# EdwardsLabProjects/sequence-alignment-tools

Measured on AMD Instinct MI355X. Metric: Gbases/s scanned, 100k×20-mer primers k≤2, 3 Gbp DB at 1/2/4/8 GPUs, higher is better.
Workload: dtype u32

## Files before the change

### sequence-alignment-tools_amd/csrc/pm_api.cpp

```cpp
#include <algorithm>
#include <climits>
#include <cstdio>
#include <cstring>
#include <memory>
#include <new>
#include <chrono>
#include <thread>
#include <unordered_map>

#include "pm_internal.h"
#include "pm_iupac.h"
#include "pm_seed.h"
#include "pm_pair.h"

using namespace pm;

namespace pm {
void Alphabet::set_raw() {
  size = 256;
  for (int i = 0; i < 256; ++i) { ch[i] = (uint8_t)i; nch[i] = i; present[i] = true; }
}
void Alphabet::set_table(const uint8_t *table, int len) {
  size = len;
  for (int i = 0; i < 256; ++i) { ch[i] = 0; nch[i] = -1; present[i] = true; }
// ... 1406 lines not shown
extern "C" int pm_reset(pm_handle *h) {
  if (!h) return PM_E_INVALID;
  drain_spec(h);
  if (h->scan_pending) { (void)hipStreamSynchronize(h->stream); h->scan_pending = false; }
  h->carry.clear(); h->land_n = h->land_pos = 0; h->next_begin = 0;
  std::fill(h->lasthit.begin(), h->lasthit.end(), 0);
  h->halves_fresh = true;
  h->last_count = 0;
  h->scan_mode = 0;
  return count_clear(h);
}

extern "C" void pm_destroy(pm_handle *h) {
  if (!h) return;
  (void)hipSetDevice(h->cfg.device);
  free_device(h);
  delete h;
}

extern "C" const char *pm_last_error(const pm_handle *h) { return h ? h->err.c_str() : g_create_error.c_str(); }
extern "C" int pm_selected_semantics(const pm_handle *h) { return h && h->inited ? h->sem : PM_E_INVALID; }
extern "C" int pm_selected_kernel(const pm_handle *h) { return h && h->inited ? h->kern : PM_E_INVALID; }

static const char *pair_schedule_name(const ScanGeometry &g) {
  return g.work_map == PAIR_MAP_XCD_SUPERCHUNK ? "xcd-superchunk" : g.work_map == PAIR_MAP_XCD ? "xcd" : "superchunk";
}

extern "C" int pm_describe(const pm_handle *h, char *buf, size_t buflen) {
  if (!h || !buf || !h->inited) return PM_E_INVALID;
  if (h->kern == PM_KERNEL_SEED && h->short_only)
    snprintf(buf, buflen, "kernel=pm_short_edit_scan+pm_edits_verify for %zu patterns of 16..19 characters (tiles=%d, tests=%d) fields=2-of-4 x 4 bases, displaced by |d| <= %d window=16 chunk=%lld nchunks=%d grid=%d block=%d",
             h->nshort, (int)h->shd.tiles.size(), h->shd.k == 2 ? SHORT_NTESTS : 2, h->shd.k, (long long)h->geo.seg_len, h->geo.nseg, h->geo.blocks, h->geo.threads);
  else if (h->kern == PM_KERNEL_SEED && !h->pair.empty()) {
    snprintf(buf, buflen, "kernel=pm_pair_scan tiles=%d combos=%d fields=2-of-4 x 5 bases window=20 row_slots=%d chunk=%lld nchunks=%d grid=%d block=%d lds=%d schedule=%s",
             (int)h->pair.size(), h->pair[0].ncombos, h->pair[0].stride, (long long)h->geo.seg_len, h->geo.nseg, h->geo.blocks, h->geo.threads, PAIR_LDS_BYTES,
             pair_schedule_name(h->geo));
    if (h->nlong) {
      int wide = 0;
      for (const PairDevice &d : h->pair) wide += d.wide ? 1 : 0;
      const size_t at = strlen(buf);
      if (at < buflen) snprintf(buf + at, buflen - at, " with %zu patterns of 33..64 characters (pm_pair_verify_wide, wide tiles=%d)", h->nlong, wide);
    }
    if (h->nrest) {
      const size_t at = strlen(buf);
      if (at < buflen) snprintf(buf + at, buflen - at, " + %s for %zu patterns the seed plan does not take", bitpar_kernel_name(h->scan_k, h->scan_indels), h->nrest);
    }
  }
  else if (h->kern == PM_KERNEL_SEED && h->edits_dev && h->epair_on) {
    snprintf(buf, buflen, "kernel=pm_pair_edit_scan+pm_pair_edit_resolve+pm_edits_verify tiles=1 tests=14 fields=2-of-4 x 5 bases, displaced by |d| <= 2 window=20 row_slots=%d slot_patterns=2 chunk=%lld nchunks=%d grid=%d block=%d lds=%d schedule=%s",
             h->epair.stride, (long long)h->geo.seg_len, h->geo.nseg, h->geo.blocks, h->geo.threads, PAIR_LDS_BYTES, pair_schedule_name(h->geo));
    if (h->nrest) {
      const size_t at = strlen(buf);
      if (at < buflen) snprintf(buf + at, buflen - at, " + %s for %zu patterns the seed plan does not take", bitpar_kernel_name(h->scan_k, h->scan_indels), h->nrest);
    }
  }
  else if (h->kern == PM_KERNEL_SEED) {
    snprintf(buf, buflen, "kernel=%s tiles=%d combos=%d pieces=%d-of-%d x %d bases window=%d slots=%zu chunk=%lld nchunks=%d grid=%d block=%d lds=%d",
             h->sd.edits && h->sd.edit_tabulated ? "pm_edit_scan+pm_edits_verify" : h->sd.edits ? "pm_seed_scan+pm_edits_verify" :
             h->sd.halves && h->sd.half_ranked ? "pm_half_scan+pm_half_verify" : "pm_seed_scan", 1 + (int)h->sd_more.size(), h->sd.ncombos, h->sd.r, h->sd.k + h->sd.r, h->sd.pb, h->sd.Lw, h->sd.nslots, (long long)h->geo.seg_len, h->geo.nseg,
             h->geo.blocks, h->geo.threads, SEED_LDS_BYTES);
    if (h->nlong_exact) {
      int wide = h->sd.wide ? 1 : 0;
      for (const SeedDevice &d : h->sd_more) wide += d.wide ? 1 : 0;
      const size_t at = strlen(buf);
      if (at < buflen) snprintf(buf + at, buflen - at, " with %zu patterns of 33..64 characters (wide rows, wide tiles=%d)", h->nlong_exact, wide);
    }
    if (h->nrest) {
      const size_t at = strlen(buf);
      if (at < buflen) snprintf(buf + at, buflen - at, " + %s for %zu patterns the seed plan does not take", bitpar_kernel_name(h->scan_k, h->scan_indels), h->nrest);
    }
  }
  if (h->kern == PM_KERNEL_SEED && h->nshort && !h->short_only) {
    const size_t at = strlen(buf);
    if (at < buflen) snprintf(buf + at, buflen - at, " + pm_short_edit_scan for %zu patterns of 16..19 characters (tiles=%d, tests=%d)", h->nshort, (int)h->shd.tiles.size(), h->shd.k == 2 ? SHORT_NTESTS : 2);
  }
  if (h->kern == PM_KERNEL_SEED && h->nssub) {
    const size_t at = strlen(buf);
    if (at < buflen) snprintf(buf + at, buflen - at, " + pm_short_sub_scan for %zu patterns of 16..19 characters (tiles=%d, pairs=%d)", h->nssub, (int)h->ssd.tiles.size(), h->ssd.ncombos);
  }
  if (h->kern == PM_KERNEL_SEED) return PM_OK;
  else
    snprintf(buf, buflen, "kernel=%s tiles=%d lanes_per_tile=64 words_per_lane=%d seg_len=%lld nseg=%d grid=%d block=%d",
             bitpar_kernel_name(h->scan_k, h->scan_indels), h->bp.ntiles, BP_WPL, (long long)h->geo.seg_len, h->geo.nseg,
// ... 1736 lines not shown
```

### sequence-alignment-tools_amd/csrc/pm_pair.h

```cpp
#pragma once
#include <array>
#include <cstdint>
#include <string>
#include <vector>

#include "pm_internal.h"
#include "pm_workmap.h"

namespace pm {

constexpr int PAIR_THREADS = 1024;
constexpr int PAIR_WAVES = PAIR_THREADS / 64;
constexpr int PAIR_MAX_COMBOS = 6;
constexpr int PAIR_BITMAP_WORDS = 32768;
constexpr int PAIR_QUEUE = 128;
constexpr int PAIR_LDS_BYTES = PAIR_BITMAP_WORDS * 4 + PAIR_WAVES * PAIR_QUEUE * 16;
static_assert(PAIR_LDS_BYTES <= 163840, "160 KiB of LDS per workgroup");
constexpr int PAIR_XCD_MIN_CHUNKS = 5 * 256;

struct PairTables {
  int k = 0, maxlen = 0, ncombos = 0, eos_code = -1, stride = 0;
  bool ascii = false;
  bool wide = false;
  int fa[PAIR_MAX_COMBOS] = {}, fb[PAIR_MAX_COMBOS] = {};
  std::vector<uint32_t> image;
  std::vector<uint64_t> slots;
  std::vector<uint32_t> row_base;
  std::vector<uint32_t> first_pat;
  std::vector<uint32_t> order;
  std::vector<uint32_t> olist;
  size_t first_off[PAIR_MAX_COMBOS] = {};
  std::vector<uint64_t> pat40;
  std::vector<uint8_t> pat_len;
  std::vector<uint32_t> pat_id;
  std::vector<uint8_t> pat_codes;
  std::vector<uint32_t> pat_zone;
};

struct PairDevice {
  int k = 0, maxlen = 0, ncombos = 0, eos_code = -1, stride = 0;
  bool ascii = false;
  bool wide = false;
  int fa[PAIR_MAX_COMBOS] = {}, fb[PAIR_MAX_COMBOS] = {};
  size_t first_off[PAIR_MAX_COMBOS] = {};
  size_t np = 0;
  uint64_t *slots = nullptr;
  uint32_t *image = nullptr, *row_base = nullptr, *first_pat = nullptr, *order = nullptr, *olist = nullptr, *pat_id = nullptr;
  uint64_t *pat40 = nullptr;
  uint8_t *pat_len = nullptr, *pat_codes = nullptr;
  uint32_t *pat_zone = nullptr;
  int viol_level = 0;
  Knobs knobs;
};

constexpr int PAIR_MAX_LEN = 32, PAIR_MAX_LEN_WIDE = 64;
std::string pair_build(const std::vector<Pattern> &pats, const std::vector<uint32_t> &ids, const Alphabet &alpha, int k,
                       int eos_code, PairTables *out, int stride_knob = 0, int slot_patterns = 3, int max_len = PAIR_MAX_LEN);
hipError_t pair_upload(const PairTables &t, PairDevice *d, hipStream_t st);
void pair_free(PairDevice *d);
ScanGeometry pair_geometry(const PairDevice &d, int64_t begin, int64_t end);
constexpr size_t PAIR_SUSPECT_BYTES = 16;
hipError_t pair_launch(const PairDevice &d, const uint8_t *d_text, const uint32_t *d_packed, int64_t n, int64_t begin, int64_t end,
                       pm_hit *d_out, unsigned long long *d_counter, uint64_t cap, void *d_susp, unsigned long long *d_susp_count, uint64_t susp_cap,
                       hipStream_t st, ScanGeometry *geo_out, unsigned long long *d_stats = nullptr, int floor_mode = 0,
                       uint64_t *seed_out = nullptr, unsigned long long *seed_count = nullptr, uint64_t seed_cap = 0);

}
```

### sequence-alignment-tools_amd/csrc/pm_pair.hip

```cpp
#include "pm_bits.h"
#include "pm_internal.h"
#include "pm_pair.h"
#include "pm_verify.h"
#include "pm_workmap.h"

#include <algorithm>
#include <cstring>
#include <thread>
#include <type_traits>
#include <utility>

namespace pm {

namespace {

constexpr int WAVES = PAIR_WAVES;
constexpr uint32_t F20 = 0xfffffu;
constexpr uint32_t WHAT_REST = 8u, WHAT_ALL = 16u;
__device__ __host__ __forceinline__ uint64_t slot_pack(uint32_t o1, uint32_t o2, uint32_t o3, bool walk) {
  return (uint64_t)o1 | ((uint64_t)o2 << 20) | ((uint64_t)o3 << 40) | ((uint64_t)(walk ? 8 : 0) << 60);
}

struct PairArgs {
  const uint8_t *text;
  int64_t n, begin, end;
  const uint32_t *packed;
  int64_t npacked;
  int64_t chunk0, chunk_len;
  int nchunks, ncombos, group;
  int work_map;
  int k, eos_code, debug;
  int stride;
  int fa[PAIR_MAX_COMBOS], fb[PAIR_MAX_COMBOS];
  const uint32_t *image;
  const uint2 *slots;
  const uint32_t *row_base;
  const uint32_t *first_pat, *order;
  const uint32_t *olist;
  uint32_t first_off[PAIR_MAX_COMBOS];
  uint32_t np;
  const uint2 *pat40;
  const uint8_t *pat_len;
  const uint32_t *pat_id;
  const uint8_t *pat_codes;
  const uint32_t *pat_zone;
  int viol_level;
  pm_hit *out;
  unsigned long long *counter;
  unsigned long long cap;
  uint4 *susp;
  unsigned long long *susp_count;
  unsigned long long susp_cap;
  uint64_t *seed_out;
  unsigned long long *seed_count;
  unsigned long long seed_cap;
  unsigned long long *stats;
};

typedef __attribute__((address_space(3))) uint32_t lds_u32;
typedef uint32_t u32x4 __attribute__((ext_vector_type(4)));
typedef uint32_t u32x2 __attribute__((ext_vector_type(2)));
typedef __attribute__((address_space(3))) u32x4 lds_u128;
__device__ __forceinline__ lds_u128 *lds128(uint32_t addr) { return reinterpret_cast<lds_u128 *>((uintptr_t)addr); }
__device__ __forceinline__ lds_u32 *lds32(uint32_t addr) { return reinterpret_cast<lds_u32 *>((uintptr_t)addr); }

__device__ __host__ __forceinline__ uint32_t field_of(uint64_t W, int j) { return (uint32_t)(W >> (10 * j)) & 0x3ffu; }
__device__ __host__ __forceinline__ void other_fields(int a, int b, int *c, int *d) {
  int o[2], t = 0;
  for (int j = 0; j < 4; ++j) if (j != a && j != b) o[t++] = j;
  *c = o[0]; *d = o[1];
}


template <int OFF>
__device__ __forceinline__ uint32_t wbits(uint32_t wlo, uint32_t whi) {
  static_assert(OFF >= 0 && OFF < 48, "window offset");
  if constexpr (OFF == 0) return wlo;
  else if constexpr (OFF < 32) return __builtin_amdgcn_alignbit(whi, wlo, OFF);
  else return whi >> (OFF - 32);
}
template <int NB, int T>
__device__ __forceinline__ uint32_t mism(uint32_t p, uint32_t wlo, uint32_t whi) {
  static_assert(T >= -2 && T + NB <= 22, "text base outside the window");
  const uint32_t x = p ^ wbits<2 * (T + 2)>(wlo, whi);
  return (x | (x >> 1)) & (NB == 5 ? 0x155u : 0x55555u);
}
enum { REG_L = 0, REG_M = 1, REG_R = 2 };
template <int NB>
__device__ __forceinline__ bool two_deletions(uint32_t lowm, uint32_t midm, uint32_t highm) {
  const int lo = __builtin_ctz(lowm | (1u << (2 * NB)));
  const int hi = 31 - __builtin_clz(highm | 1u);
  const uint32_t between = ((1u << hi) - 1u) & ~((2u << lo) - 1u);
  return (midm & between) == 0;
}
template <int KIND, int NB, int T0, int BASE, int DSP, int BUDGET>
// ... 90 lines not shown
__device__ __host__ __forceinline__ int edit_variant_table(int var) { return var == 0 ? 0 : (var <= 3 ? 1 : (var <= 8 ? 2 : (var == 9 ? 3 : (var <= 12 ? 4 : 5)))); }


template <int CW>
__device__ __forceinline__ void pair_resolve(const PairArgs &a, const VerifyStage &vs, int combo, uint32_t rank, uint32_t what, uint32_t wo, int64_t p, pm_hit *first, bool *have) {
  const uint32_t *fp = a.first_pat + a.first_off[combo];
  const uint32_t *ord = a.order + (size_t)combo * a.np;
  const uint32_t *ol = a.olist + (size_t)combo * a.np;
  const uint32_t t0 = fp[rank], t1 = fp[rank + 1];
  pm_hit hh;
  auto take = [&](bool ok) __attribute__((always_inline)) {
    const bool extra = ok && *have;
    if (ok && !*have) { *first = hh; *have = true; }
    pair_emit(a, vs, extra, hh);
  };
  for (uint32_t j = 0; j < 3; ++j)
    take(((what >> j) & 1u) && t0 + j < t1 && pair_verify<5, CW>(a, combo, p, ord[t0 + j], &hh));
  if (what & (WHAT_REST | WHAT_ALL)) {
    for (uint32_t t = t0 + ((what & WHAT_ALL) ? 0u : 3u); t < t1; ++t)
      take(sym_distance(ol[t] ^ wo) <= a.k && pair_verify<5, CW>(a, combo, p, ord[t], &hh));
  }
}

template <int CW>
__device__ __forceinline__ void pair_verify_body(const PairArgs &a) {
  unsigned long long n = *a.susp_count;
  if (n > a.susp_cap) n = a.susp_cap;
  verify_staged(a, n, [&](unsigned long long i, const VerifyStage &vs, pm_hit *first) __attribute__((always_inline)) {
    bool have = false;
    const uint4 r = a.susp[i];
    const uint64_t pw = ((uint64_t)r.w << 32) | r.z;
    if (r.x != 0xffffffffu) {
      const int combo = (int)((pw >> 40) & 7u);
      const uint32_t key = r.x, wo = r.y, row = key & 0x7fffu, bit = key >> 15;
      const uint32_t wd = a.image[(size_t)combo * PAIR_BITMAP_WORDS + row];
      if ((wd >> bit) & 1u) {
        const uint32_t lr = (uint32_t)__popc(wd & ((1u << bit) - 1u));
        const uint32_t rank = a.row_base[(size_t)combo * (PAIR_BITMAP_WORDS + 1) + row] + lr;
        uint32_t what = WHAT_ALL;
        if (lr < (uint32_t)a.stride - 1u) {
          const uint2 sl = a.slots[((size_t)combo * PAIR_BITMAP_WORDS + row) * (size_t)a.stride + lr];
          const uint64_t S = ((uint64_t)sl.y << 32) | sl.x;
          what = (sym_distance(((uint32_t)S ^ wo) & F20) <= a.k ? 1u : 0u) | (sym_distance(((uint32_t)(S >> 20) ^ wo) & F20) <= a.k ? 2u : 0u) |
                 (sym_distance(((uint32_t)(S >> 40) ^ wo) & F20) <= a.k ? 4u : 0u) | ((sl.y >> 31) ? WHAT_REST : 0u);
        }
        pair_resolve<CW>(a, vs, combo, rank, what, wo, (int64_t)(pw & 0xffffffffffull), first, &have);
      }
    }
    return have && !(a.debug & 16);
  });
}
__global__ __launch_bounds__(256) void pm_pair_verify(PairArgs a) { pair_verify_body<32>(a); }
__global__ __launch_bounds__(256) void pm_pair_verify_wide(PairArgs a) { pair_verify_body<64>(a); }

template <int A, int B, int DSP = 0, int FLOOR = 0>
__device__ __forceinline__ void pair_scan_body(const PairArgs &a, const int combo, const int cj, const int variant = 0) {
  constexpr int C = (A != 0 && B != 0) ? 0 : ((A != 1 && B != 1) ? 1 : 2);
  constexpr int D = (A != 3 && B != 3) ? 3 : ((A != 2 && B != 2) ? 2 : 1);
  static_assert(A < B && C < D && C != A && C != B && D != A && D != B, "fields");
  const int lane = threadIdx.x & 63;
  const int wave = __builtin_amdgcn_readfirstlane((int)(threadIdx.x >> 6));
  const int64_t sub = a.chunk_len / WAVES;
  const int64_t ws = (a.chunk0 + cj) * a.chunk_len + (int64_t)wave * sub;
  int64_t own_lo = ws > a.begin ? ws : a.begin;
  int64_t own_hi = ws + sub;
  if (own_hi > a.end) own_hi = a.end;
  if (own_hi > a.n) own_hi = a.n;
  if (own_lo < 19) own_lo = 19;
  if (own_lo >= own_hi) return;

  const uint32_t stride = (uint32_t)a.stride, kmax = stride - 1u;
  const char *slots = reinterpret_cast<const char *>(a.slots + (size_t)combo * PAIR_BITMAP_WORDS * stride);
  uint32_t carry1, carry2;
  {
    const uint32_t pk = load_packed(a.packed, a.npacked, ws - 32 + 16 * (lane & 1));
    carry2 = __builtin_amdgcn_readlane(pk, 0);
    carry1 = __builtin_amdgcn_readlane(pk, 1);
  }
  const uint32_t QB = PAIR_BITMAP_WORDS * 4 + (uint32_t)wave * (PAIR_QUEUE * 16);
  int qn = 0;
  uint32_t keep = 0;

  const int64_t pre_hi = FLOOR == 3 ? own_hi + 1024 : own_hi;
  uint32_t q0 = load_packed(a.packed, a.npacked, ws + 16 * lane);
  uint32_t q1 = ws + 1024 < pre_hi ? load_packed(a.packed, a.npacked, ws + 1024 + 16 * lane) : 0u;
  uint32_t q2 = ws + 2048 < pre_hi ? load_packed(a.packed, a.npacked, ws + 2048 + 16 * lane) : 0u;
  uint32_t q3 = ws + 3072 < pre_hi ? load_packed(a.packed, a.npacked, ws + 3072 + 16 * lane) : 0u;
  const uint32_t *pk_wave = a.packed + (ws >> 4);
  uint32_t pf_idx = 4096u / 16u + (uint32_t)lane;

  const int negk1 = -(a.k + 1);

  unsigned long long blk_at = 0;
  uint32_t blk_left = 0, blk_next = 0;
  auto flush = [&]() __attribute__((always_inline)) {
    int done = 0;
    while (done < qn) {
      if (blk_left == 0) {
        const uint32_t want = max((uint32_t)(qn - done), blk_next);
        unsigned long long base = 0;
        if (lane == 0) base = atomicAdd(a.susp_count, (unsigned long long)want);
        blk_at = ((unsigned long long)__builtin_amdgcn_readfirstlane((uint32_t)(base >> 32)) << 32) | __builtin_amdgcn_readfirstlane((uint32_t)base);
        blk_left = want;
        blk_next = min(2u * max(want, 64u), 4096u);
      }
// ... 13 lines not shown
    blk_left = 0;
  };
  auto enqueue = [&](bool mine, uint32_t key, uint32_t wo, uint32_t prel) __attribute__((always_inline)) {
    const unsigned long long bal = __ballot(mine);
    if (bal == 0) return;
    if (a.debug & 1) { keep ^= key; return; }
    if (mine) {
      const int s_ = qn + (int)__builtin_amdgcn_mbcnt_hi((uint32_t)(bal >> 32), __builtin_amdgcn_mbcnt_lo((uint32_t)bal, 0));
      u32x4 q;
      q.x = key; q.y = wo; q.z = prel; q.w = 0;
      *lds128(QB + 16 * (uint32_t)s_) = q;
    }
    qn += __popcll(bal);
    if (qn >= 64) flush();
  };

  auto key_of = [&](auto WIN, uint32_t prev2, uint32_t prev1, uint32_t cur) __attribute__((always_inline)) -> uint32_t {
    constexpr int I = decltype(WIN)::value;
    const uint32_t X = bits_at<2 * I + 26 + 10 * A - 2 - 2 * DSP>(prev2, prev1, cur);
    if constexpr (B == A + 1 && DSP == 0) return X;
    else { const uint32_t Y = bits_at<2 * I + 26 + 10 * B - 12>(prev2, prev1, cur); return (X & 0xffcu) | (Y & ~0xffcu); }
  };

#ifndef PM_PAIR_NR
#define PM_PAIR_NR 6
#endif
  constexpr int NR = PM_PAIR_NR;
  static_assert(NR % 2 == 0 && NR >= 4 && NR <= 12, "ring size");
  uint32_t P = 0;
  uint32_t pu1 = 0, pu2 = 0, pu3 = 0, cu1 = 0, cu2 = 0, cu3 = 0;
  uint32_t tagbase = 0xfffffff0u;
  u32x2 e_sl[NR];
  uint32_t e_key[NR], e_wo[NR], e_rel[NR], e_okm[NR], e_wd[NR];
  uint32_t e_hi[FLOOR >= 2 ? NR : 1];
  for (int d = 0; d < (FLOOR >= 2 ? NR : 1); ++d) e_hi[d] = 0;
#pragma unroll
  for (int d = 0; d < NR; ++d) { e_sl[d].x = 0; e_sl[d].y = 0; e_key[d] = e_wo[d] = e_rel[d] = e_okm[d] = e_wd[d] = 0; }
  uint32_t m5v, f20v, rowmask;
  asm volatile("v_mov_b32 %0, 0x55555\n v_mov_b32 %1, 0xfffff\n v_mov_b32 %2, 0x7fff" : "=v"(m5v), "=v"(f20v), "=v"(rowmask));

  auto round = [&](auto PHASE) __attribute__((always_inline)) {
    constexpr int PH = decltype(PHASE)::value, LD = (PH + NR - 1) % NR;
    if constexpr (FLOOR == 3) {
      const uint32_t lo = e_wo[PH], hi = e_hi[PH];
      const int d1 = edit_cost<A, B, DSP, true>(e_sl[PH].x & f20v, lo, hi) - 3;
      const int d2 = edit_cost<A, B, DSP, true>(__builtin_amdgcn_alignbit(e_sl[PH].y, e_sl[PH].x, 20) & f20v, lo, hi) - 3;
      const bool susp = (int)(((uint32_t)(d1 | d2) | e_sl[PH].y) & e_okm[PH]) < 0;
      enqueue(susp, lo, hi, ((e_rel[PH] >> 4) << 10) + 16u * (uint32_t)lane + (e_rel[PH] & 15u));
    } else if constexpr (FLOOR == 2) {
      constexpr int OC = 4 + 10 * C;
      const uint32_t lo = e_wo[PH], hi = e_hi[PH];
      uint32_t T[5];
      static_for<5>([&](auto SI) __attribute__((always_inline)) { constexpr int si = decltype(SI)::value; T[si] = __builtin_amdgcn_alignbit(hi, lo, OC + 2 * (si - 2)) & f20v; });
      auto score = [&](uint32_t o) __attribute__((always_inline)) -> int {
        uint32_t m[5];
        static_for<5>([&](auto SI) __attribute__((always_inline)) { constexpr int si = decltype(SI)::value; const uint32_t x = o ^ T[si]; m[si] = (x | (x >> 1)) & m5v; });
        const int c0 = __popc(m[2]), c1 = __popc(m[2] & m[3]) + 1, c1n = __popc(m[2] & m[1]) + 1;
        const int c2 = __popc(m[2] & m[3] & m[4]) + 2, c2n = __popc(m[2] & m[1] & m[0]) + 2;
        return min(min(c0, min(c1, c1n)), min(c2, c2n)) - 3;
      };
      const int d1 = score(e_sl[PH].x & f20v), d2 = score(__builtin_amdgcn_alignbit(e_sl[PH].y, e_sl[PH].x, 20) & f20v);
      const bool susp = (int)(((uint32_t)(d1 | d2) | e_sl[PH].y) & e_okm[PH]) < 0;
      enqueue(susp, e_key[PH], lo, ((e_rel[PH] >> 4) << 10) + 16u * (uint32_t)lane + (e_rel[PH] & 15u));
    } else {
      const uint32_t w = e_wo[PH];
      const uint32_t x1 = e_sl[PH].x ^ w, x2 = __builtin_amdgcn_alignbit(e_sl[PH].y, e_sl[PH].x, 20) ^ w, x3 = (e_sl[PH].y >> 8) ^ w;
      const int d1 = __popc((x1 | (x1 >> 1)) & m5v) + negk1;
      const int d2 = __popc((x2 | (x2 >> 1)) & m5v) + negk1;
      const int d3 = __popc((x3 | (x3 >> 1)) & m5v) + negk1;
      const bool susp = (int)(((uint32_t)(d1 | d2 | d3) | e_sl[PH].y) & e_okm[PH]) < 0;
      enqueue(susp, e_key[PH], w, ((e_rel[PH] >> 4) << 10) + 16u * (uint32_t)lane + (e_rel[PH] & 15u));
    }
    {
      const uint32_t bit = e_key[LD] >> 15;
      const uint32_t lr = min((uint32_t)__popc(__builtin_amdgcn_ubfe(e_wd[LD], 0, bit)), kmax);
      const uint32_t off = (__umul24(e_key[LD] & rowmask, stride) + lr) << 3;
      e_sl[LD] = *reinterpret_cast<const u32x2 *>(slots + off);
    }
    {
      uint32_t i;
      asm("v_ffbl_b32 %0, %1" : "=v"(i) : "v"(P));
      P &= P - 1u;
      const uint32_t okm = ~i;
      const bool cb = (i & 16u) != 0;
      const uint32_t j2 = i + i;
      const uint32_t u1 = cb ? cu1 : pu1, u2 = cb ? cu2 : pu2, u3 = cb ? cu3 : pu3;
      const uint32_t wlo = __builtin_amdgcn_alignbit(u2, u1, j2), whi = __builtin_amdgcn_alignbit(u3, u2, j2);
      auto from = [&](int O) __attribute__((always_inline)) -> uint32_t { return O == 0 ? wlo : (O == 10 ? wlo >> 10 : __builtin_amdgcn_alignbit(whi, wlo, 20)); };
      uint32_t key, wo;
      if constexpr (FLOOR != 0) {
        constexpr int OA = 4 + 10 * A - 2 * DSP, OB = 4 + 10 * B - 10, OCC = 4 + 10 * C, ODD = 4 + 10 * D - 10;
        key = (__builtin_amdgcn_alignbit(whi, wlo, OA) & 0x3ffu) | (__builtin_amdgcn_alignbit(whi, wlo, OB) & 0xffc00u);
        if constexpr (FLOOR >= 2) { wo = wlo; e_hi[PH] = whi; }
        else wo = (__builtin_amdgcn_alignbit(whi, wlo, OCC) & 0x3ffu) | (__builtin_amdgcn_alignbit(whi, wlo, ODD) & 0xffc00u);
      } else {
      if constexpr (B == A + 1) key = from(10 * A) & f20v; else key = (from(10 * A) & 0x3ffu) | (from(10 * B - 10) & 0xffc00u);
      if constexpr (D == C + 1) wo = from(10 * C) & f20v; else wo = (from(10 * C) & 0x3ffu) | (from(10 * D - 10) & 0xffc00u);
      }
      key &= (uint32_t)((int)okm >> 31);
      e_key[PH] = key; e_wo[PH] = wo; e_okm[PH] = okm;
      e_rel[PH] = tagbase + i;
      e_wd[PH] = *lds32((key & rowmask) << 2);
    }
  };
  int ph = 0;
  int quiet = NR + 1;
  auto two_rounds = [&]() __attribute__((always_inline)) {
    bool done = false;
    static_for<NR / 2>([&](auto Q) __attribute__((always_inline)) {
      constexpr int q = decltype(Q)::value;
      if (!done && ph == q) {
        round(std::integral_constant<int, 2 * q>()); round(std::integral_constant<int, 2 * q + 1>());
        ph = q + 1 == NR / 2 ? 0 : q + 1;
        done = true;
      }
    });
  };

  const bool stats = (a.debug & 32) != 0 && a.stats != nullptr;
  uint32_t st_blocks = 0, st_rounds = 0, st_hits = 0;
  int64_t bb = ws;
  const int rmin = (a.debug >> 8) & 15 ? (a.debug >> 8) & 15 : 2;
  while (bb < own_hi) {
    const uint32_t cur = q0;
    q0 = q1; q1 = q2; q2 = q3;
    if (bb + 4096 < pre_hi) q3 = pk_wave[pf_idx];
    pf_idx += 64u;
    const uint32_t prev1 = __builtin_amdgcn_update_dpp(carry1, cur, 0x138, 0xf, 0xf, false);
    const uint32_t prev2 = __builtin_amdgcn_update_dpp(carry2, prev1, 0x138, 0xf, 0xf, false);
    carry2 = __builtin_amdgcn_readlane(cur, 62);
    carry1 = __builtin_amdgcn_readlane(cur, 63);
    uint32_t own = 0xffffu;
    if (bb < own_lo || bb + 1024 > own_hi) {
      const int64_t pbase = bb + 16 * lane;
      const int64_t lo = own_lo - pbase, hi = own_hi - pbase;
// ... 225 lines not shown
  for (size_t j = 0; j < np; ++j) {
    const int L = (int)pats[j].s.size();
    if (L < 20 || L > max_len) return max_len > PAIR_MAX_LEN ? "the pair plan needs patterns of 20..64 characters" : "the pair plan needs patterns of 20..32 characters";
    t.wide = t.wide || L > PAIR_MAX_LEN;
  }
  const size_t CW = t.wide ? 64 : 32;
  t.pat40.resize(np); t.pat_len.resize(np); t.pat_id.resize(np); t.pat_codes.assign(np * CW, 0); t.pat_zone.assign(np * (CW / 32), 0);
  for (size_t j = 0; j < np; ++j) {
    const std::string &s = pats[j].s;
    const int L = (int)s.size();
    uint64_t w = 0;
    for (int i = 0; i < 20; ++i) {
      const int b2 = base2((unsigned char)s[L - 20 + i]);
      if (b2 < 0) return "pattern with characters other than A,C,G,T";
      w |= (uint64_t)b2 << (2 * i);
    }
    for (int i = 0; i < L; ++i) {
      if (base2((unsigned char)s[i]) < 0) return "pattern with characters other than A,C,G,T";
      t.pat_codes[j * CW + i] = (uint8_t)alpha.nch[(unsigned char)s[i]];
    }
    t.pat40[j] = w; t.pat_len[j] = (uint8_t)L; t.pat_id[j] = ids[j];
    {
      const int es = std::max(0, std::min(L, pats[j].esb)), ee = std::max(0, std::min(L, pats[j].eeb));
      uint64_t z = 0;
      for (int i = 0; i < L; ++i) if (i < es || i >= L - ee) z |= 1ull << i;
      t.pat_zone[j * (CW / 32)] = (uint32_t)z;
      if (t.wide) t.pat_zone[j * 2 + 1] = (uint32_t)(z >> 32);
    }
    t.maxlen = std::max(t.maxlen, L);
  }
  if (k == 1) { t.ncombos = 2; t.fa[0] = 0; t.fb[0] = 1; t.fa[1] = 2; t.fb[1] = 3; }
  else { t.ncombos = 0; for (int x = 0; x < 4; ++x) for (int y = x + 1; y < 4; ++y) { t.fa[t.ncombos] = x; t.fb[t.ncombos] = y; ++t.ncombos; } }
  const int C = t.ncombos;
  t.stride = stride_knob >= 2 && stride_knob <= 33 ? stride_knob : (np <= 230000 ? 12 : (np <= 300000 ? 14 : 16));
  const size_t ST = (size_t)t.stride, KMAX = ST - 1;
  t.image.assign((size_t)C * PAIR_BITMAP_WORDS, 0);
  t.order.assign((size_t)C * np, 0);
  t.olist.assign((size_t)C * np, 0);
  t.slots.assign((size_t)C * PAIR_BITMAP_WORDS * ST, 0);
  t.row_base.assign((size_t)C * (PAIR_BITMAP_WORDS + 1), 0);
  std::vector<std::vector<uint32_t>> fp(C);
  auto build_combo = [&](int ci) {
    const int fa = t.fa[ci], fb = t.fb[ci];
    int fc, fd;
    other_fields(fa, fb, &fc, &fd);
    std::vector<uint64_t> srt(np);
    for (size_t j = 0; j < np; ++j) {
      const uint32_t key = field_of(t.pat40[j], fa) | (field_of(t.pat40[j], fb) << 10);
      const uint32_t bitpos = ((key & 0x7fffu) << 5) | (key >> 15);
      srt[j] = ((uint64_t)bitpos << 32) | (uint64_t)j;
    }
    std::sort(srt.begin(), srt.end());
    uint32_t *img = &t.image[(size_t)ci * PAIR_BITMAP_WORDS];
    uint32_t *ord = &t.order[(size_t)ci * np];
    uint32_t *ol = &t.olist[(size_t)ci * np];
    uint64_t *slot = &t.slots[(size_t)ci * PAIR_BITMAP_WORDS * ST];
    uint32_t *rb = &t.row_base[(size_t)ci * (PAIR_BITMAP_WORDS + 1)];
    std::vector<uint32_t> &f = fp[ci];
    f.reserve(np + 1);
    for (size_t r = 0; r < (size_t)PAIR_BITMAP_WORDS; ++r) slot[r * ST + KMAX] = slot_pack(0, 0, 0, true);
    uint32_t cur_row = 0, in_row = 0;
    for (size_t j = 0; j < np;) {
      const uint32_t bitpos = (uint32_t)(srt[j] >> 32);
      size_t j2 = j;
      while (j2 < np && (uint32_t)(srt[j2] >> 32) == bitpos) ++j2;
      const uint32_t row = bitpos >> 5;
      while (cur_row < row) { rb[++cur_row] = (uint32_t)f.size(); in_row = 0; }
      img[row] |= 1u << (bitpos & 31u);
      f.push_back((uint32_t)j);
      uint32_t o[3] = {0, 0, 0};
      for (size_t q = j; q < j2; ++q) {
        const uint32_t pi = (uint32_t)srt[q];
        ord[q] = pi;
        ol[q] = field_of(t.pat40[pi], fc) | (field_of(t.pat40[pi], fd) << 10);
        if (q - j < SP) o[q - j] = field_of(t.pat40[pi], fc) | (field_of(t.pat40[pi], fd) << 10);
      }
      for (size_t q = std::min(j2 - j, SP); q < 3; ++q) o[q] = o[0];
      if (in_row < KMAX) slot[(size_t)row * ST + in_row] = slot_pack(o[0], o[1], o[2], j2 - j > SP);
      ++in_row;
      j = j2;
    }
    while (cur_row < (uint32_t)PAIR_BITMAP_WORDS) rb[++cur_row] = (uint32_t)f.size();
    f.push_back((uint32_t)np);
  };
  if (np * (size_t)C < 20000) for (int ci = 0; ci < C; ++ci) build_combo(ci);
  else {
    std::vector<std::thread> th;
    for (int ci = 0; ci < C; ++ci) th.emplace_back([&, ci]() { build_combo(ci); });
    for (std::thread &x : th) x.join();
  }
  for (int ci = 0; ci < C; ++ci) {
    t.first_off[ci] = t.first_pat.size();
    t.first_pat.insert(t.first_pat.end(), fp[ci].begin(), fp[ci].end());
  }
  return "";
}

hipError_t pair_upload(const PairTables &t, PairDevice *d, hipStream_t st) {
  pair_free(d);
  d->k = t.k; d->maxlen = t.maxlen; d->ncombos = t.ncombos; d->eos_code = t.eos_code; d->ascii = t.ascii; d->wide = t.wide; d->np = t.pat40.size(); d->stride = t.stride;
  for (int c = 0; c < PAIR_MAX_COMBOS; ++c) { d->fa[c] = t.fa[c]; d->fb[c] = t.fb[c]; d->first_off[c] = t.first_off[c]; }
  auto up = [&](const void *src, size_t bytes, void **dst) -> hipError_t {
    hipError_t e = hipMalloc(dst, bytes ? bytes : 16);
    if (e != hipSuccess) return e;
    return bytes ? hipMemcpyAsync(*dst, src, bytes, hipMemcpyHostToDevice, st) : hipSuccess;
  };
  hipError_t e;
  if ((e = up(t.image.data(), t.image.size() * 4, (void **)&d->image)) != hipSuccess) return e;
  if ((e = up(t.slots.data(), t.slots.size() * 8, (void **)&d->slots)) != hipSuccess) return e;
  if ((e = up(t.row_base.data(), t.row_base.size() * 4, (void **)&d->row_base)) != hipSuccess) return e;
  if ((e = up(t.first_pat.data(), t.first_pat.size() * 4, (void **)&d->first_pat)) != hipSuccess) return e;
  if ((e = up(t.order.data(), t.order.size() * 4, (void **)&d->order)) != hipSuccess) return e;
  if ((e = up(t.olist.data(), t.olist.size() * 4, (void **)&d->olist)) != hipSuccess) return e;
  if ((e = up(t.pat40.data(), t.pat40.size() * 8, (void **)&d->pat40)) != hipSuccess) return e;
  if ((e = up(t.pat_len.data(), t.pat_len.size(), (void **)&d->pat_len)) != hipSuccess) return e;
  if ((e = up(t.pat_id.data(), t.pat_id.size() * 4, (void **)&d->pat_id)) != hipSuccess) return e;
  if ((e = up(t.pat_codes.data(), t.pat_codes.size(), (void **)&d->pat_codes)) != hipSuccess) return e;
  if ((e = up(t.pat_zone.data(), t.pat_zone.size() * 4, (void **)&d->pat_zone)) != hipSuccess) return e;
  hipFuncAttributes fa;
  if ((e = hipFuncGetAttributes(&fa, reinterpret_cast<const void *>(pm_pair_scan))) != hipSuccess) return e;
  if (fa.sharedSizeBytes != 0) return hipErrorInvalidConfiguration;
  if ((e = hipFuncSetAttribute(reinterpret_cast<const void *>(pm_pair_scan), hipFuncAttributeMaxDynamicSharedMemorySize, PAIR_LDS_BYTES)) != hipSuccess) return e;
  return hipStreamSynchronize(st);
}

void pair_free(PairDevice *d) {
  void *ptrs[] = {d->image, d->slots, d->row_base, d->first_pat, d->order, d->olist, d->pat_id, d->pat40, d->pat_len, d->pat_codes, d->pat_zone};
  for (void *p : ptrs) if (p) (void)hipFree(p);
  *d = PairDevice();
}

ScanGeometry pair_geometry(const PairDevice &d, int64_t begin, int64_t end) {
  ScanGeometry g;
  int64_t chunk = 1 << 19;
  const int64_t range = end - begin;
  if (range / ((int64_t)1 << 21) * d.ncombos >= 256 * 16) chunk = (int64_t)1 << 21;
  else if (range / ((int64_t)1 << 20) * d.ncombos >= 256 * 16) chunk = (int64_t)1 << 20;
  if (d.knobs.seed_chunk >= 1024 * WAVES) chunk = d.knobs.seed_chunk / (1024 * WAVES) * (1024 * WAVES);
  g.seg_len = chunk;
  const int64_t c_lo = begin / chunk, c_hi = end > begin ? (end - 1) / chunk : c_lo - 1;
  g.nseg = (int)(c_hi - c_lo + 1);
  g.threads = PAIR_THREADS;
  g.blocks = g.nseg * d.ncombos;
  g.work_map = g.nseg >= PAIR_XCD_MIN_CHUNKS ? PAIR_MAP_XCD_SUPERCHUNK : PAIR_MAP_SUPERCHUNK;
  if (d.knobs.pair_map >= 0) g.work_map = d.knobs.pair_map;
  return g;
}

hipError_t pair_launch(const PairDevice &d, const uint8_t *d_text, const uint32_t *d_packed, int64_t n, int64_t begin, int64_t end,
                       pm_hit *d_out, unsigned long long *d_counter, uint64_t cap, void *d_susp, unsigned long long *d_susp_count, uint64_t susp_cap,
                       hipStream_t st, ScanGeometry *geo_out, unsigned long long *d_stats, int floor_mode,
                       uint64_t *seed_out, unsigned long long *seed_count, uint64_t seed_cap) {
  if (!d_packed) return hipErrorInvalidValue;
  if (end > n) end = n;
  if (floor_mode && (d.k != 2 || d.ncombos != 6)) return hipErrorInvalidValue;
  if (floor_mode == 3 && (!seed_out || !seed_count)) return hipErrorInvalidValue;
  ScanGeometry g = pair_geometry(d, begin, end);
  if (floor_mode) {
    g.blocks = g.nseg * 14;
    if (d.knobs.pair_map < 0) g.work_map = PAIR_MAP_SUPERCHUNK;
  }
  if (geo_out) *geo_out = g;
  if (g.blocks <= 0 || d.np == 0) return hipSuccess;
  PairArgs a;
  memset(&a, 0, sizeof(a));
  a.text = d_text; a.n = n; a.begin = begin; a.end = end;
  a.packed = d_packed; a.npacked = (n + 15) / 16;
  a.chunk_len = g.seg_len; a.chunk0 = begin / g.seg_len; a.nchunks = g.nseg; a.ncombos = d.ncombos;
  a.group = 256;
  if (d.knobs.seed_group > 0) a.group = d.knobs.seed_group;
  a.work_map = g.work_map;
  a.k = d.k; a.eos_code = d.eos_code;
  a.debug = d.knobs.seed_debug;
  for (int c = 0; c < PAIR_MAX_COMBOS; ++c) { a.fa[c] = d.fa[c]; a.fb[c] = d.fb[c]; a.first_off[c] = (uint32_t)d.first_off[c]; }
  a.stride = d.stride;
  a.image = d.image; a.slots = reinterpret_cast<const uint2 *>(d.slots); a.row_base = d.row_base; a.first_pat = d.first_pat; a.order = d.order; a.olist = d.olist;
  a.np = (uint32_t)d.np;
  a.pat40 = reinterpret_cast<const uint2 *>(d.pat40); a.pat_len = d.pat_len; a.pat_id = d.pat_id; a.pat_codes = d.pat_codes; a.pat_zone = d.pat_zone; a.viol_level = d.viol_level;
  a.out = d_out; a.counter = d_counter; a.cap = cap;
  if (!d_susp || !d_susp_count) return hipErrorInvalidValue;
  a.susp = reinterpret_cast<uint4 *>(d_susp); a.susp_count = d_susp_count; a.susp_cap = susp_cap;
  a.stats = d_stats;
  a.seed_out = seed_out; a.seed_count = seed_count; a.seed_cap = seed_cap;
  if (floor_mode) {
    a.ncombos = 14;
    hipError_t fe;
    if (floor_mode == 1) {
      if ((fe = hipFuncSetAttribute(reinterpret_cast<const void *>(pm_pair_edit_scan<1>), hipFuncAttributeMaxDynamicSharedMemorySize, PAIR_LDS_BYTES)) != hipSuccess) return fe;
      hipLaunchKernelGGL(pm_pair_edit_scan<1>, dim3(g.blocks), dim3(PAIR_THREADS), PAIR_LDS_BYTES, st, a);
    } else if (floor_mode == 2) {
      if ((fe = hipFuncSetAttribute(reinterpret_cast<const void *>(pm_pair_edit_scan<2>), hipFuncAttributeMaxDynamicSharedMemorySize, PAIR_LDS_BYTES)) != hipSuccess) return fe;
      hipLaunchKernelGGL(pm_pair_edit_scan<2>, dim3(g.blocks), dim3(PAIR_THREADS), PAIR_LDS_BYTES, st, a);
    } else {
      if ((fe = hipFuncSetAttribute(reinterpret_cast<const void *>(pm_pair_edit_scan<3>), hipFuncAttributeMaxDynamicSharedMemorySize, PAIR_LDS_BYTES)) != hipSuccess) return fe;
      hipLaunchKernelGGL(pm_pair_edit_scan<3>, dim3(g.blocks), dim3(PAIR_THREADS), PAIR_LDS_BYTES, st, a);
      if ((fe = hipGetLastError()) != hipSuccess) return fe;
      hipLaunchKernelGGL(pm_pair_edit_resolve, dim3(16384), dim3(256), 0, st, a);
    }
    return hipGetLastError();
  }
  hipLaunchKernelGGL(pm_pair_scan, dim3(g.blocks), dim3(PAIR_THREADS), PAIR_LDS_BYTES, st, a);
  hipError_t ce = hipGetLastError();
  if (ce != hipSuccess) return ce;
  if (d.wide) hipLaunchKernelGGL(pm_pair_verify_wide, dim3(32768), dim3(256), 0, st, a);
  else hipLaunchKernelGGL(pm_pair_verify, dim3(32768), dim3(256), 0, st, a);
  return hipGetLastError();
}

// ... 2 lines not shown
```

Baseline: 216.5.

## Group pair-filter slot rows into 64-key rows with density-derived stride

Makes the pair-scan slot table use rows covering two bitmap dwords (64 keys) for the main scan, loading both dwords with a single 64-bit LDS read and computing the local rank across them. The row stride now comes from a binomial overflow model of the measured key density instead of a fixed pattern-count table. Overflow markers are set only on rows that actually overflow. The intent is to cut slot-table size and overflow fallbacks (WHAT_ALL/rest paths), in exchange for extra popcount/select work per candidate and a wider LDS read.

```diff
diff --git a/sequence-alignment-tools_amd/csrc/pm_api.cpp b/sequence-alignment-tools_amd/csrc/pm_api.cpp
--- a/sequence-alignment-tools_amd/csrc/pm_api.cpp
+++ b/sequence-alignment-tools_amd/csrc/pm_api.cpp
@@ -1462,8 +1462,8 @@
     snprintf(buf, buflen, "kernel=pm_short_edit_scan+pm_edits_verify for %zu patterns of 16..19 characters (tiles=%d, tests=%d) fields=2-of-4 x 4 bases, displaced by |d| <= %d window=16 chunk=%lld nchunks=%d grid=%d block=%d",
              h->nshort, (int)h->shd.tiles.size(), h->shd.k == 2 ? SHORT_NTESTS : 2, h->shd.k, (long long)h->geo.seg_len, h->geo.nseg, h->geo.blocks, h->geo.threads);
   else if (h->kern == PM_KERNEL_SEED && !h->pair.empty()) {
-    snprintf(buf, buflen, "kernel=pm_pair_scan tiles=%d combos=%d fields=2-of-4 x 5 bases window=20 row_slots=%d chunk=%lld nchunks=%d grid=%d block=%d lds=%d schedule=%s",
-             (int)h->pair.size(), h->pair[0].ncombos, h->pair[0].stride, (long long)h->geo.seg_len, h->geo.nseg, h->geo.blocks, h->geo.threads, PAIR_LDS_BYTES,
+    snprintf(buf, buflen, "kernel=pm_pair_scan tiles=%d combos=%d fields=2-of-4 x 5 bases window=20 row_slots=%d row_keys=%d chunk=%lld nchunks=%d grid=%d block=%d lds=%d schedule=%s",
+             (int)h->pair.size(), h->pair[0].ncombos, h->pair[0].stride, h->pair[0].row_keys, (long long)h->geo.seg_len, h->geo.nseg, h->geo.blocks, h->geo.threads, PAIR_LDS_BYTES,
              pair_schedule_name(h->geo));
     if (h->nlong) {
       int wide = 0;
@@ -1477,8 +1477,8 @@
     }
   }
   else if (h->kern == PM_KERNEL_SEED && h->edits_dev && h->epair_on) {
-    snprintf(buf, buflen, "kernel=pm_pair_edit_scan+pm_pair_edit_resolve+pm_edits_verify tiles=1 tests=14 fields=2-of-4 x 5 bases, displaced by |d| <= 2 window=20 row_slots=%d slot_patterns=2 chunk=%lld nchunks=%d grid=%d block=%d lds=%d schedule=%s",
-             h->epair.stride, (long long)h->geo.seg_len, h->geo.nseg, h->geo.blocks, h->geo.threads, PAIR_LDS_BYTES, pair_schedule_name(h->geo));
+    snprintf(buf, buflen, "kernel=pm_pair_edit_scan+pm_pair_edit_resolve+pm_edits_verify tiles=1 tests=14 fields=2-of-4 x 5 bases, displaced by |d| <= 2 window=20 row_slots=%d row_keys=%d slot_patterns=2 chunk=%lld nchunks=%d grid=%d block=%d lds=%d schedule=%s",
+             h->epair.stride, h->epair.row_keys, (long long)h->geo.seg_len, h->geo.nseg, h->geo.blocks, h->geo.threads, PAIR_LDS_BYTES, pair_schedule_name(h->geo));
     if (h->nrest) {
       const size_t at = strlen(buf);
       if (at < buflen) snprintf(buf + at, buflen - at, " + %s for %zu patterns the seed plan does not take", bitpar_kernel_name(h->scan_k, h->scan_indels), h->nrest);
diff --git a/sequence-alignment-tools_amd/csrc/pm_pair.h b/sequence-alignment-tools_amd/csrc/pm_pair.h
--- a/sequence-alignment-tools_amd/csrc/pm_pair.h
+++ b/sequence-alignment-tools_amd/csrc/pm_pair.h
@@ -5,6 +5,7 @@
 #include <vector>
 
 #include "pm_internal.h"
+#include "pm_pair_rows.h"
 #include "pm_workmap.h"
 
 namespace pm {
@@ -20,6 +21,7 @@
 
 struct PairTables {
   int k = 0, maxlen = 0, ncombos = 0, eos_code = -1, stride = 0;
+  int row_keys = 0;
   bool ascii = false;
   bool wide = false;
   int fa[PAIR_MAX_COMBOS] = {}, fb[PAIR_MAX_COMBOS] = {};
@@ -38,7 +40,7 @@
 };
 
 struct PairDevice {
-  int k = 0, maxlen = 0, ncombos = 0, eos_code = -1, stride = 0;
+  int k = 0, maxlen = 0, ncombos = 0, eos_code = -1, stride = 0, row_keys = 0;
   bool ascii = false;
   bool wide = false;
   int fa[PAIR_MAX_COMBOS] = {}, fb[PAIR_MAX_COMBOS] = {};
diff --git a/sequence-alignment-tools_amd/csrc/pm_pair.hip b/sequence-alignment-tools_amd/csrc/pm_pair.hip
--- a/sequence-alignment-tools_amd/csrc/pm_pair.hip
+++ b/sequence-alignment-tools_amd/csrc/pm_pair.hip
@@ -1,6 +1,7 @@
 #include "pm_bits.h"
 #include "pm_internal.h"
 #include "pm_pair.h"
+#include "pm_pair_rows.h"
 #include "pm_verify.h"
 #include "pm_workmap.h"
 
@@ -31,6 +32,7 @@
   int work_map;
   int k, eos_code, debug;
   int stride;
+  int row_keys;
   int fa[PAIR_MAX_COMBOS], fb[PAIR_MAX_COMBOS];
   const uint32_t *image;
   const uint2 *slots;
@@ -61,6 +63,8 @@
 typedef uint32_t u32x4 __attribute__((ext_vector_type(4)));
 typedef uint32_t u32x2 __attribute__((ext_vector_type(2)));
 typedef __attribute__((address_space(3))) u32x4 lds_u128;
+typedef __attribute__((address_space(3))) u32x2 lds_u64;
+[[maybe_unused]] __device__ __forceinline__ lds_u64 *lds64(uint32_t addr) { return reinterpret_cast<lds_u64 *>((uintptr_t)addr); }
 __device__ __forceinline__ lds_u128 *lds128(uint32_t addr) { return reinterpret_cast<lds_u128 *>((uintptr_t)addr); }
 __device__ __forceinline__ lds_u32 *lds32(uint32_t addr) { return reinterpret_cast<lds_u32 *>((uintptr_t)addr); }
 
@@ -217,14 +221,17 @@
     const uint64_t pw = ((uint64_t)r.w << 32) | r.z;
     if (r.x != 0xffffffffu) {
       const int combo = (int)((pw >> 40) & 7u);
-      const uint32_t key = r.x, wo = r.y, row = key & 0x7fffu, bit = key >> 15;
-      const uint32_t wd = a.image[(size_t)combo * PAIR_BITMAP_WORDS + row];
-      if ((wd >> bit) & 1u) {
-        const uint32_t lr = (uint32_t)__popc(wd & ((1u << bit) - 1u));
-        const uint32_t rank = a.row_base[(size_t)combo * (PAIR_BITMAP_WORDS + 1) + row] + lr;
+      const uint32_t key = r.x, wo = r.y;
+      const int rk = a.row_keys;
+      const uint32_t *img = a.image + (size_t)combo * PAIR_BITMAP_WORDS;
+      const uint32_t d0 = pair_row_dword(key, rk);
+      const uint32_t lo = img[d0], hi = rk == 64 ? img[d0 + 1] : 0u;
+      if (((((key & 0x7fffu) == d0) ? lo : hi) >> (key >> 15)) & 1u) {
+        const uint32_t lr = pair_local_rank(lo, hi, key, rk);
+        const uint32_t rank = a.row_base[(size_t)combo * (PAIR_BITMAP_WORDS + 1) + d0] + lr;
         uint32_t what = WHAT_ALL;
-        if (lr < (uint32_t)a.stride - 1u) {
-          const uint2 sl = a.slots[((size_t)combo * PAIR_BITMAP_WORDS + row) * (size_t)a.stride + lr];
+        if (pair_own_slot(lr, pair_row_count(lo, hi, rk), (uint32_t)a.stride)) {
+          const uint2 sl = a.slots[(size_t)combo * pair_rows(rk) * (size_t)a.stride + pair_slot_index(key, lr, (uint32_t)a.stride, rk)];
           const uint64_t S = ((uint64_t)sl.y << 32) | sl.x;
           what = (sym_distance(((uint32_t)S ^ wo) & F20) <= a.k ? 1u : 0u) | (sym_distance(((uint32_t)(S >> 20) ^ wo) & F20) <= a.k ? 2u : 0u) |
                  (sym_distance(((uint32_t)(S >> 40) ^ wo) & F20) <= a.k ? 4u : 0u) | ((sl.y >> 31) ? WHAT_REST : 0u);
@@ -254,8 +261,10 @@
   if (own_lo < 19) own_lo = 19;
   if (own_lo >= own_hi) return;
 
-  const uint32_t stride = (uint32_t)a.stride, kmax = stride - 1u;
-  const char *slots = reinterpret_cast<const char *>(a.slots + (size_t)combo * PAIR_BITMAP_WORDS * stride);
+  constexpr int RK = FLOOR == 3 ? PAIR_EDIT_ROW_KEYS : PAIR_ROW_KEYS;
+  const uint32_t stride = (uint32_t)a.stride;
+  const uint32_t rowbytes = stride * (RK == 64 ? 4u : 8u);
+  const char *slots = reinterpret_cast<const char *>(a.slots + (size_t)combo * pair_rows(RK) * stride);
   uint32_t carry1, carry2;
   {
     const uint32_t pk = load_packed(a.packed, a.npacked, ws - 32 + 16 * (lane & 1));
@@ -335,12 +344,15 @@
   uint32_t tagbase = 0xfffffff0u;
   u32x2 e_sl[NR];
   uint32_t e_key[NR], e_wo[NR], e_rel[NR], e_okm[NR], e_wd[NR];
+  uint32_t e_wh[RK == 64 ? NR : 1];
+  for (int d = 0; d < (RK == 64 ? NR : 1); ++d) e_wh[d] = 0;
   uint32_t e_hi[FLOOR >= 2 ? NR : 1];
   for (int d = 0; d < (FLOOR >= 2 ? NR : 1); ++d) e_hi[d] = 0;
 #pragma unroll
   for (int d = 0; d < NR; ++d) { e_sl[d].x = 0; e_sl[d].y = 0; e_key[d] = e_wo[d] = e_rel[d] = e_okm[d] = e_wd[d] = 0; }
   uint32_t m5v, f20v, rowmask;
-  asm volatile("v_mov_b32 %0, 0x55555\n v_mov_b32 %1, 0xfffff\n v_mov_b32 %2, 0x7fff" : "=v"(m5v), "=v"(f20v), "=v"(rowmask));
+  if constexpr (RK == 64) asm volatile("v_mov_b32 %0, 0x55555\n v_mov_b32 %1, 0xfffff\n v_mov_b32 %2, 0x7ffe" : "=v"(m5v), "=v"(f20v), "=v"(rowmask));
+  else asm volatile("v_mov_b32 %0, 0x55555\n v_mov_b32 %1, 0xfffff\n v_mov_b32 %2, 0x7fff" : "=v"(m5v), "=v"(f20v), "=v"(rowmask));
 
   auto round = [&](auto PHASE) __attribute__((always_inline)) {
     constexpr int PH = decltype(PHASE)::value, LD = (PH + NR - 1) % NR;
@@ -375,9 +387,8 @@
       enqueue(susp, e_key[PH], w, ((e_rel[PH] >> 4) << 10) + 16u * (uint32_t)lane + (e_rel[PH] & 15u));
     }
     {
-      const uint32_t bit = e_key[LD] >> 15;
-      const uint32_t lr = min((uint32_t)__popc(__builtin_amdgcn_ubfe(e_wd[LD], 0, bit)), kmax);
-      const uint32_t off = (__umul24(e_key[LD] & rowmask, stride) + lr) << 3;
+      const uint32_t sr = pair_slot_in_row(pair_local_rank(e_wd[LD], e_wh[RK == 64 ? LD : 0], e_key[LD], RK), stride);
+      const uint32_t off = __umul24(e_key[LD] & rowmask, rowbytes) + (sr << 3);
       e_sl[LD] = *reinterpret_cast<const u32x2 *>(slots + off);
     }
     {
@@ -403,7 +414,8 @@
       key &= (uint32_t)((int)okm >> 31);
       e_key[PH] = key; e_wo[PH] = wo; e_okm[PH] = okm;
       e_rel[PH] = tagbase + i;
-      e_wd[PH] = *lds32((key & rowmask) << 2);
+      if constexpr (RK == 64) { const u32x2 w2 = *lds64((key & rowmask) << 2); e_wd[PH] = w2.x; e_wh[PH] = w2.y; }
+      else e_wd[PH] = *lds32((key & rowmask) << 2);
     }
   };
   int ph = 0;
@@ -695,12 +707,25 @@
   if (k == 1) { t.ncombos = 2; t.fa[0] = 0; t.fb[0] = 1; t.fa[1] = 2; t.fb[1] = 3; }
   else { t.ncombos = 0; for (int x = 0; x < 4; ++x) for (int y = x + 1; y < 4; ++y) { t.fa[t.ncombos] = x; t.fb[t.ncombos] = y; ++t.ncombos; } }
   const int C = t.ncombos;
-  t.stride = stride_knob >= 2 && stride_knob <= 33 ? stride_knob : (np <= 230000 ? 12 : (np <= 300000 ? 14 : 16));
-  const size_t ST = (size_t)t.stride, KMAX = ST - 1;
   t.image.assign((size_t)C * PAIR_BITMAP_WORDS, 0);
+  size_t distinct = 0;
+  for (int ci = 0; ci < C; ++ci) {
+    uint32_t *img = &t.image[(size_t)ci * PAIR_BITMAP_WORDS];
+    for (size_t j = 0; j < np; ++j) {
+      const uint32_t key = field_of(t.pat40[j], t.fa[ci]) | (field_of(t.pat40[j], t.fb[ci]) << 10);
+      img[key & 0x7fffu] |= 1u << (key >> 15);
+    }
+    for (size_t r = 0; r < (size_t)PAIR_BITMAP_WORDS; ++r) distinct += pair_popc(img[r]);
+  }
+  t.row_keys = SP == 2 ? PAIR_EDIT_ROW_KEYS : PAIR_ROW_KEYS;
+  const int RK = t.row_keys;
+  const double density = (double)distinct / ((double)C * 1048576.0);
+  t.stride = stride_knob >= PAIR_ROW_SLOTS_MIN && stride_knob <= PAIR_ROW_SLOTS_MAX ? stride_knob
+                                                                                     : pair_default_stride(RK, density, RK == 64 ? PAIR_OVERFLOW_BOUND : PAIR_OVERFLOW_BOUND_32);
+  const size_t ST = (size_t)t.stride, ROWS = pair_rows(RK);
   t.order.assign((size_t)C * np, 0);
   t.olist.assign((size_t)C * np, 0);
-  t.slots.assign((size_t)C * PAIR_BITMAP_WORDS * ST, 0);
+  t.slots.assign((size_t)C * ROWS * ST, 0);
   t.row_base.assign((size_t)C * (PAIR_BITMAP_WORDS + 1), 0);
   std::vector<std::vector<uint32_t>> fp(C);
   auto build_combo = [&](int ci) {
@@ -717,19 +742,23 @@
     uint32_t *img = &t.image[(size_t)ci * PAIR_BITMAP_WORDS];
     uint32_t *ord = &t.order[(size_t)ci * np];
     uint32_t *ol = &t.olist[(size_t)ci * np];
-    uint64_t *slot = &t.slots[(size_t)ci * PAIR_BITMAP_WORDS * ST];
+    uint64_t *slot = &t.slots[(size_t)ci * ROWS * ST];
     uint32_t *rb = &t.row_base[(size_t)ci * (PAIR_BITMAP_WORDS + 1)];
     std::vector<uint32_t> &f = fp[ci];
     f.reserve(np + 1);
-    for (size_t r = 0; r < (size_t)PAIR_BITMAP_WORDS; ++r) slot[r * ST + KMAX] = slot_pack(0, 0, 0, true);
-    uint32_t cur_row = 0, in_row = 0;
+    auto row_dwords = [&](uint32_t key, uint32_t *lo, uint32_t *hi) { const uint32_t d0 = pair_row_dword(key, RK); *lo = img[d0]; *hi = RK == 64 ? img[d0 + 1] : 0u; };
+    for (uint32_t d0 = 0; d0 < (uint32_t)PAIR_BITMAP_WORDS; d0 += (uint32_t)RK / 32u) {
+      uint32_t lo, hi;
+      row_dwords(d0, &lo, &hi);
+      if (pair_row_overflows(pair_row_count(lo, hi, RK), (uint32_t)ST)) slot[(size_t)pair_row_of(d0, RK) * ST + ST - 1] = slot_pack(0, 0, 0, true);
+    }
+    uint32_t cur_row = 0;
     for (size_t j = 0; j < np;) {
       const uint32_t bitpos = (uint32_t)(srt[j] >> 32);
       size_t j2 = j;
       while (j2 < np && (uint32_t)(srt[j2] >> 32) == bitpos) ++j2;
-      const uint32_t row = bitpos >> 5;
-      while (cur_row < row) { rb[++cur_row] = (uint32_t)f.size(); in_row = 0; }
-      img[row] |= 1u << (bitpos & 31u);
+      const uint32_t row = bitpos >> 5, key = row | ((bitpos & 31u) << 15);
+      while (cur_row < row) rb[++cur_row] = (uint32_t)f.size();
       f.push_back((uint32_t)j);
       uint32_t o[3] = {0, 0, 0};
       for (size_t q = j; q < j2; ++q) {
@@ -739,8 +768,10 @@
         if (q - j < SP) o[q - j] = field_of(t.pat40[pi], fc) | (field_of(t.pat40[pi], fd) << 10);
       }
       for (size_t q = std::min(j2 - j, SP); q < 3; ++q) o[q] = o[0];
-      if (in_row < KMAX) slot[(size_t)row * ST + in_row] = slot_pack(o[0], o[1], o[2], j2 - j > SP);
-      ++in_row;
+      uint32_t lo, hi;
+      row_dwords(key, &lo, &hi);
+      const uint32_t lr = pair_local_rank(lo, hi, key, RK);
+      if (pair_own_slot(lr, pair_row_count(lo, hi, RK), (uint32_t)ST)) slot[pair_slot_index(key, lr, (uint32_t)ST, RK)] = slot_pack(o[0], o[1], o[2], j2 - j > SP);
       j = j2;
     }
     while (cur_row < (uint32_t)PAIR_BITMAP_WORDS) rb[++cur_row] = (uint32_t)f.size();
@@ -761,7 +792,7 @@
 
 hipError_t pair_upload(const PairTables &t, PairDevice *d, hipStream_t st) {
   pair_free(d);
-  d->k = t.k; d->maxlen = t.maxlen; d->ncombos = t.ncombos; d->eos_code = t.eos_code; d->ascii = t.ascii; d->wide = t.wide; d->np = t.pat40.size(); d->stride = t.stride;
+  d->k = t.k; d->maxlen = t.maxlen; d->ncombos = t.ncombos; d->eos_code = t.eos_code; d->ascii = t.ascii; d->wide = t.wide; d->np = t.pat40.size(); d->stride = t.stride; d->row_keys = t.row_keys;
   for (int c = 0; c < PAIR_MAX_COMBOS; ++c) { d->fa[c] = t.fa[c]; d->fb[c] = t.fb[c]; d->first_off[c] = t.first_off[c]; }
   auto up = [&](const void *src, size_t bytes, void **dst) -> hipError_t {
     hipError_t e = hipMalloc(dst, bytes ? bytes : 16);
@@ -818,6 +849,7 @@
   if (end > n) end = n;
   if (floor_mode && (d.k != 2 || d.ncombos != 6)) return hipErrorInvalidValue;
   if (floor_mode == 3 && (!seed_out || !seed_count)) return hipErrorInvalidValue;
+  if (d.row_keys != (floor_mode == 3 ? PAIR_EDIT_ROW_KEYS : PAIR_ROW_KEYS)) return hipErrorInvalidValue;
   ScanGeometry g = pair_geometry(d, begin, end);
   if (floor_mode) {
     g.blocks = g.nseg * 14;
@@ -836,7 +868,7 @@
   a.k = d.k; a.eos_code = d.eos_code;
   a.debug = d.knobs.seed_debug;
   for (int c = 0; c < PAIR_MAX_COMBOS; ++c) { a.fa[c] = d.fa[c]; a.fb[c] = d.fb[c]; a.first_off[c] = (uint32_t)d.first_off[c]; }
-  a.stride = d.stride;
+  a.stride = d.stride; a.row_keys = d.row_keys;
   a.image = d.image; a.slots = reinterpret_cast<const uint2 *>(d.slots); a.row_base = d.row_base; a.first_pat = d.first_pat; a.order = d.order; a.olist = d.olist;
   a.np = (uint32_t)d.np;
   a.pat40 = reinterpret_cast<const uint2 *>(d.pat40); a.pat_len = d.pat_len; a.pat_id = d.pat_id; a.pat_codes = d.pat_codes; a.pat_zone = d.pat_zone; a.viol_level = d.viol_level;
diff --git a/sequence-alignment-tools_amd/csrc/pm_pair_rows.h b/sequence-alignment-tools_amd/csrc/pm_pair_rows.h
--- /dev/null
+++ b/sequence-alignment-tools_amd/csrc/pm_pair_rows.h
@@ -0,0 +1,80 @@
+#pragma once
+
+#ifndef PM_HD
+#if defined(__HIPCC__)
+#define PM_HD __host__ __device__
+#else
+#define PM_HD
+#endif
+#endif
+
+#ifndef PM_PAIR_ROW_KEYS
+#define PM_PAIR_ROW_KEYS 64
+#endif
+#ifndef PM_PAIR_EDIT_ROW_KEYS
+#define PM_PAIR_EDIT_ROW_KEYS 32
+#endif
+
+namespace pm {
+
+constexpr int PAIR_ROW_KEYS = PM_PAIR_ROW_KEYS;
+constexpr int PAIR_EDIT_ROW_KEYS = PM_PAIR_EDIT_ROW_KEYS;
+static_assert((PAIR_ROW_KEYS == 32 || PAIR_ROW_KEYS == 64) && (PAIR_EDIT_ROW_KEYS == 32 || PAIR_EDIT_ROW_KEYS == 64), "a row is one or two bitmap dwords");
+constexpr int PAIR_ROW_SLOTS_MIN = 2, PAIR_ROW_SLOTS_MAX = 65;
+
+PM_HD inline unsigned pair_popc(unsigned x) { return (unsigned)__builtin_popcount(x); }
+PM_HD inline unsigned pair_bits_below(unsigned x, unsigned bit) {
+#if defined(__HIP_DEVICE_COMPILE__)
+  return __builtin_amdgcn_ubfe(x, 0u, bit);
+#else
+  return x & ((1u << bit) - 1u);
+#endif
+}
+PM_HD inline unsigned pair_select(unsigned m, unsigned a, unsigned b) {
+#if defined(__HIP_DEVICE_COMPILE__)
+  unsigned r;
+  asm("v_bfi_b32 %0, %1, %2, %3" : "=v"(r) : "v"(m), "v"(a), "v"(b));
+  return r;
+#else
+  return (a & m) | (b & ~m);
+#endif
+}
+
+PM_HD inline unsigned pair_rows(int rk) { return rk == 64 ? 16384u : 32768u; }
+PM_HD inline unsigned pair_row_of(unsigned key, int rk) { return rk == 64 ? (key & 0x7fffu) >> 1 : key & 0x7fffu; }
+PM_HD inline unsigned pair_row_dword(unsigned key, int rk) { return rk == 64 ? key & 0x7ffeu : key & 0x7fffu; }
+PM_HD inline unsigned pair_row_pos(unsigned key, int rk) { return (rk == 64 ? 32u * (key & 1u) : 0u) + (key >> 15); }
+
+PM_HD inline unsigned pair_local_rank(unsigned lo, unsigned hi, unsigned key, int rk) {
+  if (rk != 64) return pair_popc(pair_bits_below(lo, key >> 15));
+  const unsigned m = 0u - (key & 1u);
+  return pair_popc(pair_bits_below(pair_select(m, hi, lo), key >> 15)) + pair_popc(lo & m);
+}
+PM_HD inline unsigned pair_row_count(unsigned lo, unsigned hi, int rk) { return pair_popc(lo) + (rk == 64 ? pair_popc(hi) : 0u); }
+
+PM_HD inline bool pair_own_slot(unsigned lr, unsigned count, unsigned stride) { return lr + 1u < stride || count <= stride; }
+PM_HD inline bool pair_row_overflows(unsigned count, unsigned stride) { return count > stride; }
+PM_HD inline unsigned pair_slot_in_row(unsigned lr, unsigned stride) { const unsigned last = stride - 1u; return lr < last ? lr : last; }
+PM_HD inline unsigned pair_slot_index(unsigned key, unsigned lr, unsigned stride, int rk) { return pair_row_of(key, rk) * stride + pair_slot_in_row(lr, stride); }
+
+PM_HD inline double pair_overflow_share(int rk, double p, int stride) {
+  if (p <= 0.0 || stride > rk) return 0.0;
+  if (p >= 1.0) return (double)(rk - (stride - 1)) / (double)rk;
+  double pmf = 1.0;
+  for (int i = 0; i < rk; ++i) pmf *= 1.0 - p;
+  double beyond = 0.0;
+  for (int c = 0; c <= rk; ++c) {
+    if (c > stride) beyond += pmf * (double)(c - (stride - 1));
+    pmf *= (double)(rk - c) / (double)(c + 1) * (p / (1.0 - p));
+  }
+  return beyond / ((double)rk * p);
+}
+PM_HD inline int pair_default_stride(int rk, double p, double bound) {
+  int s = PAIR_ROW_SLOTS_MIN;
+  while (s <= rk && pair_overflow_share(rk, p, s) >= bound) ++s;
+  return s;
+}
+constexpr double PAIR_OVERFLOW_BOUND = 1e-4;
+constexpr double PAIR_OVERFLOW_BOUND_32 = 1e-3;
+
+}
```

Result: no change. 217.7, median of 6 (+0.6%).
